# zyhbili/Dual-Space-NeRF

Measured on AMD Instinct MI355X. Metric: rendered rays/sec (64 samples/ray), 512x512 frame, higher is better.
Workload: dtype split-f16x3 (3 x v_mfma_f32_32x32x16_f16 on hi/lo fp16 operand halves, f32 accumulate: f32-equivalent accuracy - parity bars of the tests: 1e-4 absolute on RGB / acc / weights against the reference; sigma 1e-4 absolute where |sigma| <= 100 and 4e-6 RELATIVE to max|sigma| above (this checkpoint: |sig

## Files before the change

dual-space-nerf_amd/csrc/dsn_field16.hip:

```cpp
#include "dsn_common.h"
#include "dsn_kernels.h"

typedef float f32x16 __attribute__((ext_vector_type(16)));
typedef _Float16 half8 __attribute__((ext_vector_type(8)));
#define MFMA16(a, b, c) __builtin_amdgcn_mfma_f32_32x32x16_f16((a), (b), (c), 0, 0, 0)

#if !defined(DSN_EXPERIMENTS) && (defined(F16_ABL) || defined(F16_SABL) || defined(F16_TIMING) || defined(F16_TRAIN_ABL))
#error "F16_ABL / F16_SABL / F16_TIMING are experiment switches (wrong results / debug counters): build with -DDSN_EXPERIMENTS"
#endif
#ifndef F16_SINCOS_OCML
#define F16_SINCOS_OCML 0
#endif
#ifndef F16_FENCE
#define F16_FENCE 0
#endif
#ifndef F16_SGB
#define F16_SGB 1
#endif
#ifndef F16_SGB_VALU
#define F16_SGB_VALU 2
#endif
#ifndef F16_SGB_DS
#define F16_SGB_DS 1
#endif
// ... 1682 lines not shown
        int off = s_base;
        for (int k = 0; k < wave; ++k) off += s_cnt[k];
        if (keep[0]) keep_list[off + __popcll(bm0 & ((1ull << lane) - 1ull))] = (int32_t)pt[0];
        if (keep[1]) keep_list[off + __popcll(bm0) + __popcll(bm1 & ((1ull << lane) - 1ull))] = (int32_t)pt[1];
    }
  }
}

void dsn_launch_screen16(const float* packed, const DsnFrameState* fs, const float* x_c, int64_t N, const int32_t* active_list,
                         const int32_t* active_count, float* sigma, int32_t* keep_list, int32_t* keep_count, float* dbg_sigma,
                         float* dbg_s1, hipStream_t st, int32_t* audit_list, int32_t* audit_count, int audit_cap) {
    if (N == 0) return;
    const char* wenv = getenv("DSN_SCREEN_WAVES");
    const int waves = wenv ? atoi(wenv) : 8;
    static const float margin = getenv("DSN_SCREEN_MARGIN") ? (float)atof(getenv("DSN_SCREEN_MARGIN")) : 0.0f;
    if (waves == 4)
        hipLaunchKernelGGL(k_screen16<4>, dim3((unsigned)std::min<int64_t>((N + 127) / 128, 2 * dsn_cu_count())), dim3(256), 0, st, packed, fs, x_c, N, active_list,
                           active_count, sigma, keep_list, keep_count, dbg_sigma, dbg_s1, margin, audit_list, audit_count, audit_cap);
    else if (waves == 2)
        hipLaunchKernelGGL(k_screen16x2, dim3((unsigned)std::min<int64_t>((N + 255) / 256, dsn_cu_count())), dim3(256), 0, st, packed, fs, x_c, N, active_list,
                           active_count, sigma, keep_list, keep_count, dbg_sigma, dbg_s1, margin, audit_list, audit_count, audit_cap);
    else
        hipLaunchKernelGGL(k_screen16<8>, dim3((unsigned)std::min<int64_t>((N + 255) / 256, dsn_cu_count())), dim3(512), 0, st, packed, fs, x_c, N, active_list,
                           active_count, sigma, keep_list, keep_count, dbg_sigma, dbg_s1, margin, audit_list, audit_count, audit_cap);
}

__global__ void __launch_bounds__(256) k_screen_audit(const int32_t* __restrict__ audit_list, const int32_t* __restrict__ audit_count,
                                                      int audit_cap, const float* __restrict__ sigma, int32_t* __restrict__ out) {
    const int n = min(*audit_count, audit_cap);
    if (blockIdx.x == 0 && threadIdx.x == 0) out[2] = n;
    for (int i = blockIdx.x * 256 + threadIdx.x; i < n; i += gridDim.x * 256) {
        const float s = sigma[audit_list[i]];
        if (s > 0.0f) { atomicAdd(out, 1); atomicMax(out + 1, __float_as_int(s)); }
    }
}
void dsn_launch_screen_audit(const int32_t* audit_list, const int32_t* audit_count, int audit_cap, const float* sigma, int32_t* out,
                             hipStream_t st) {
    hipLaunchKernelGGL(k_screen_audit, dim3(64), dim3(256), 0, st, audit_list, audit_count, audit_cap, sigma, out);
}

#define F16_SCREEN_FLOOR 0.002f
#define F16_SCREEN_CAP 0.15f
#define F16_SCREEN_HEADROOM 10.0f
__global__ void __launch_bounds__(256) k_calib_points(const float4* __restrict__ cent, int F, int64_t n, float* __restrict__ x, float box) {
    const int64_t i = (int64_t)blockIdx.x * 256 + threadIdx.x;
    if (i >= n) return;
    const float4 c = cent[(int)(i % F)];
    uint32_t h = (uint32_t)i * 2654435761u + 0x9e3779b9u;
    float o[3];
    for (int k = 0; k < 3; ++k) {
        h ^= h >> 16; h *= 0x7feb352du; h ^= h >> 15; h *= 0x846ca68bu; h ^= h >> 16;
        o[k] = ((float)(h >> 8) * (1.0f / 16777216.0f) - 0.5f) * box;
    }
    x[3 * i] = c.x + o[0]; x[3 * i + 1] = c.y + o[1]; x[3 * i + 2] = c.z + o[2];
}
#define DSN_CALIB_MIN_FRAME_LIST 65536
__global__ void __launch_bounds__(256) k_calib_points_frame(const float* __restrict__ x_c, const int32_t* __restrict__ list,
                                                             const int32_t* __restrict__ count, const float4* __restrict__ cent, int F,
                                                             int64_t n, float halo, float box, float* __restrict__ x) {
    const int64_t i = (int64_t)blockIdx.x * 256 + threadIdx.x;
    if (i >= n) return;
    const int64_t cnt = (int64_t)(*count);
    uint32_t h = (uint32_t)i * 2654435761u + 0x9e3779b9u;
    float o[3];
    for (int k = 0; k < 3; ++k) {
        h ^= h >> 16; h *= 0x7feb352du; h ^= h >> 15; h *= 0x846ca68bu; h ^= h >> 16;
        o[k] = (float)(h >> 8) * (1.0f / 16777216.0f) - 0.5f;
    }
    if (cnt < DSN_CALIB_MIN_FRAME_LIST) {
        const float4 c = cent[(int)(i % F)];
        x[3 * i] = c.x + o[0] * box; x[3 * i + 1] = c.y + o[1] * box; x[3 * i + 2] = c.z + o[2] * box;
        return;
    }
    const int64_t half = n / 2 > 0 ? n / 2 : 1;
    const int64_t k = i % half;
    const int64_t slot = (int64_t)(((__int128)k * cnt) / half) % cnt;
    const int64_t s = (int64_t)list[slot];
    const float j = i >= half ? 2.0f * halo : 0.0f;
    x[3 * i] = x_c[3 * s] + o[0] * j; x[3 * i + 1] = x_c[3 * s + 1] + o[1] * j; x[3 * i + 2] = x_c[3 * s + 2] + o[2] * j;
}
__global__ void __launch_bounds__(256) k_calib_reduce(const float* __restrict__ sg, const float* __restrict__ s1,
                                                      const float* __restrict__ sig, int64_t n, uint32_t* __restrict__ acc) {
    float d = 0.0f, t = 0.0f;
    int bad = 0;
    for (int64_t i = (int64_t)blockIdx.x * 256 + threadIdx.x; i < n; i += (int64_t)gridDim.x * 256) {
        const float a = sg[i], b = s1[i], c = sig[i];
        const float q = fabsf(a - c) / (b + 1.0f);
        if (q == q && fabsf(q) < INFINITY) {
            d = fmaxf(d, q);
            t = fmaxf(t, q - fabsf(c) / (F16_SCREEN_HEADROOM * (b + 1.0f)));
        } else ++bad;
    }
#pragma unroll
    for (int o = 32; o >= 1; o >>= 1) { d = fmaxf(d, __shfl_xor(d, o)); t = fmaxf(t, __shfl_xor(t, o)); bad += __shfl_xor(bad, o); }
    if ((threadIdx.x & 63) == 0) { atomicMax(acc, __float_as_uint(d)); atomicAdd(acc + 1, (uint32_t)bad); atomicMax(acc + 3, __float_as_uint(t)); }
}
__global__ void k_calib_finish(const uint32_t* __restrict__ acc, float* __restrict__ packed_margin, float* __restrict__ out4, float n) {
    const float d = __uint_as_float(acc[0]);
    float t = __uint_as_float(acc[3]);
    if (out4 && out4[7] > t) t = out4[7];
    float m = fmaxf(F16_SCREEN_HEADROOM * t, F16_SCREEN_FLOOR);
    if (!(m <= F16_SCREEN_CAP)) m = INFINITY;
    *packed_margin = m;
    if (out4) { out4[0] = d; out4[1] = m; out4[2] = (float)acc[1] / n; out4[3] = n; out4[5] = t; }
}
__global__ void __launch_bounds__(256) k_calib_dropped(const float* __restrict__ sg, const float* __restrict__ s1, int64_t n,
                                                       const float* __restrict__ packed_margin, uint32_t* __restrict__ acc) {
    const float m = *packed_margin;
    int c = 0;
    for (int64_t i = (int64_t)blockIdx.x * 256 + threadIdx.x; i < n; i += (int64_t)gridDim.x * 256) c += sg[i] < -(m * s1[i] + m) ? 1 : 0;
#pragma unroll
    for (int o = 32; o >= 1; o >>= 1) c += __shfl_xor(c, o);
    if ((threadIdx.x & 63) == 0 && c) atomicAdd(acc + 2, (uint32_t)c);
}
__global__ void k_calib_dropped_finish(const uint32_t* __restrict__ acc, float* __restrict__ out, float n) { out[4] = (float)acc[2] / n; }
size_t dsn_calibrate_workspace_size(int64_t n) { return 256 + dsn_align256(12 * (size_t)n) + 4 * dsn_align256(4 * (size_t)n); }
void dsn_launch_calibrate_screen(const DsnSceneView& s, float* packed, int64_t n, void* workspace, float* out4, hipStream_t st,
                                 const float* frame_x_c, const int32_t* frame_list, const int32_t* frame_count) {
    char* p = (char*)workspace;
    uint32_t* acc = (uint32_t*)p;             p += 256;
    float* x = (float*)p;                     p += dsn_align256(12 * (size_t)n);
    float* sg = (float*)p;                    p += dsn_align256(4 * (size_t)n);
    float* s1 = (float*)p;                    p += dsn_align256(4 * (size_t)n);
    float* sig = (float*)p;                   p += dsn_align256(4 * (size_t)n);
    int32_t* lst = (int32_t*)p;
    (void)hipMemsetAsync(acc, 0, 256, st);
    const char* be = getenv("DSN_CALIB_BOX");
    const float box = be ? (float)atof(be) : 0.3f;
    if (frame_x_c)
        hipLaunchKernelGGL(k_calib_points_frame, dim3((unsigned)((n + 255) / 256)), dim3(256), 0, st, frame_x_c, frame_list, frame_count,
                           s.cent_canon, s.F, n, 0.02f, box, x);
    else
        hipLaunchKernelGGL(k_calib_points, dim3((unsigned)((n + 255) / 256)), dim3(256), 0, st, s.cent_canon, s.F, n, x, box);
    dsn_launch_screen16(packed, s.frame, x, n, nullptr, nullptr, sg, lst, (int32_t*)(acc + 8), sg, s1, st, nullptr, nullptr, 0);
    dsn_launch_field(packed, s.frame, x, n, nullptr, nullptr, sig, nullptr, nullptr, st);
    hipLaunchKernelGGL(k_calib_reduce, dim3(1024), dim3(256), 0, st, sg, s1, sig, n, acc);
    hipLaunchKernelGGL(k_calib_finish, dim3(1), dim3(1), 0, st, acc, packed + OFF_SCAL + 5, out4, (float)n);
    if (out4) {
        hipLaunchKernelGGL(k_calib_dropped, dim3(1024), dim3(256), 0, st, sg, s1, n, packed + OFF_SCAL + 5, acc);
        hipLaunchKernelGGL(k_calib_dropped_finish, dim3(1), dim3(1), 0, st, acc, out4, (float)n);
    }
}
__global__ void k_set_scalar(float* p, float v) { *p = v; }
void dsn_launch_set_screen_margin(float* packed, float margin, hipStream_t st) {
    hipLaunchKernelGGL(k_set_scalar, dim3(1), dim3(1), 0, st, packed + OFF_SCAL + 5, margin);
}
void dsn_launch_set_packed_scalar(float* packed, int word, float v, hipStream_t st) {
    hipLaunchKernelGGL(k_set_scalar, dim3(1), dim3(1), 0, st, packed + OFF_SCAL + word, v);
}

#define DSN_MFMA(a, b, c) __builtin_amdgcn_mfma_f32_32x32x2f32((a), (b), (c), 0, 0, 0)
__device__ __forceinline__ float dsn_light_mlp32(const float* __restrict__ packed, int lane, const float (&in9)[10]) {
    const int half = lane >> 5;
    f32x16 h1[4], h2[4];
#pragma unroll
    for (int m = 0; m < 4; ++m) {
        f32x16 acc = rows16(packed + OFF_BLT0, m, half);
        const float4* wp = reinterpret_cast<const float4*>(packed + OFF_LT0 + m * DSN_BLK) + lane;
        const float4 w0 = wp[0], w1 = wp[64];
        acc = DSN_MFMA(w0.x, half ? in9[1] : in9[0], acc);
        acc = DSN_MFMA(w0.y, half ? in9[3] : in9[2], acc);
        acc = DSN_MFMA(w0.z, half ? in9[5] : in9[4], acc);
        acc = DSN_MFMA(w0.w, half ? in9[7] : in9[6], acc);
        acc = DSN_MFMA(w1.x, half ? in9[9] : in9[8], acc);
#pragma unroll
        for (int r = 0; r < 16; ++r) acc[r] = acc[r] > 0.0f ? acc[r] : 0.0f;
        h1[m] = acc;
    }
#pragma unroll
    for (int m = 0; m < 4; ++m) {
        f32x16 acc = rows16(packed + OFF_BLT1, m, half);
#pragma unroll
        for (int kb = 0; kb < 4; ++kb) {
            const float4* bp = reinterpret_cast<const float4*>(packed + OFF_LT1 + (m * 4 + kb) * DSN_BLK) + lane;
            const float4 c0 = bp[0], c1 = bp[64], c2 = bp[128], c3 = bp[192];
            acc = DSN_MFMA(c0.x, h1[kb][0], acc);  acc = DSN_MFMA(c0.y, h1[kb][1], acc);
            acc = DSN_MFMA(c0.z, h1[kb][2], acc);  acc = DSN_MFMA(c0.w, h1[kb][3], acc);
            acc = DSN_MFMA(c1.x, h1[kb][4], acc);  acc = DSN_MFMA(c1.y, h1[kb][5], acc);
            acc = DSN_MFMA(c1.z, h1[kb][6], acc);  acc = DSN_MFMA(c1.w, h1[kb][7], acc);
            acc = DSN_MFMA(c2.x, h1[kb][8], acc);  acc = DSN_MFMA(c2.y, h1[kb][9], acc);
            acc = DSN_MFMA(c2.z, h1[kb][10], acc); acc = DSN_MFMA(c2.w, h1[kb][11], acc);
            acc = DSN_MFMA(c3.x, h1[kb][12], acc); acc = DSN_MFMA(c3.y, h1[kb][13], acc);
            acc = DSN_MFMA(c3.z, h1[kb][14], acc); acc = DSN_MFMA(c3.w, h1[kb][15], acc);
        }
#pragma unroll
        for (int r = 0; r < 16; ++r) acc[r] = acc[r] > 0.0f ? acc[r] : 0.0f;
        h2[m] = acc;
    }
    float part = 0.0f;
#pragma unroll
    for (int m = 0; m < 4; ++m) {
        const f32x16 w = rows16(packed + OFF_WLT2, m, half);
#pragma unroll
        for (int r = 0; r < 16; ++r) part = fmaf(w[r], h2[m][r], part);
    }
    part += __shfl_xor(part, 32);
    return part + packed[OFF_SCAL + 4];
}

#define LIGHT32_THREADS 256
__global__ void __launch_bounds__(LIGHT32_THREADS, 1)
k_light(const float* __restrict__ packed, const DsnFrameState* __restrict__ fs, const float* __restrict__ n_w,
        const float* __restrict__ x_w_pts, const float* __restrict__ ray_o, const float* __restrict__ ray_d,
        const float* __restrict__ z_vals, const float* essence, int64_t N, int S,
        const int32_t* __restrict__ active_list, const int32_t* __restrict__ active_count,
        float* colour) {
    DSN_OWN_SIMD();
    const int lane = threadIdx.x & 63;
    const int wave = __builtin_amdgcn_readfirstlane(threadIdx.x >> 6);
    const int half = lane >> 5;
    const int64_t count = active_list ? (int64_t)(*active_count) : N;
    const int64_t slot0 = ((int64_t)blockIdx.x * 4 + wave) * 32;
    if (slot0 >= count) return;
    int64_t slot = slot0 + (lane & 31);
    const bool valid = slot < count;
    if (!valid) slot = count - 1;
    const int64_t pt = active_list ? (int64_t)active_list[slot] : slot;
    const int64_t ray = pt / S;

    float in9[10];
    in9[0] = n_w[3 * pt]; in9[1] = n_w[3 * pt + 1]; in9[2] = n_w[3 * pt + 2];
    float xw[3];
    const float d[3] = {ray_d[3 * ray], ray_d[3 * ray + 1], ray_d[3 * ray + 2]};
    if (x_w_pts) { xw[0] = x_w_pts[3 * pt]; xw[1] = x_w_pts[3 * pt + 1]; xw[2] = x_w_pts[3 * pt + 2]; }
    else {
        const float z = z_vals[pt];
        xw[0] = ray_o[3 * ray] + d[0] * z; xw[1] = ray_o[3 * ray + 1] + d[1] * z; xw[2] = ray_o[3 * ray + 2] + d[2] * z;
    }
    dsn_light_edit(fs->light, xw);
    in9[3] = xw[0]; in9[4] = xw[1]; in9[5] = xw[2];
    const float vn = dsn_norm3(d);
    in9[6] = dsn_div(d[0], vn); in9[7] = dsn_div(d[1], vn); in9[8] = dsn_div(d[2], vn);
    in9[9] = 0.0f;

    const float o = dsn_light_mlp32(packed, lane, in9);
    const float wgt = (o > 0.0f ? o : expm1f(o)) + 1.0f;
    if (valid && half == 0) {
        colour[3 * pt + 0] = wgt * essence[3 * pt + 0];
        colour[3 * pt + 1] = wgt * essence[3 * pt + 1];
        colour[3 * pt + 2] = wgt * essence[3 * pt + 2];
    }
}

void dsn_launch_light(const float* packed, const DsnFrameState* fs, const float* n_w, const float* x_w,
                      const float* ray_o, const float* ray_d, const float* z_vals, const float* essence, int64_t N,
                      int S, const int32_t* active_list, const int32_t* active_count, float* colour, hipStream_t st) {
    int64_t blocks = (N + 127) / 128;
    if (blocks == 0) return;
    hipLaunchKernelGGL(k_light, dim3((unsigned)blocks), dim3(LIGHT32_THREADS), 0, st, packed, fs, n_w, x_w, ray_o, ray_d,
                       z_vals, essence, N, S, active_list, active_count, colour);
}

__device__ __forceinline__ void light_block0(const char* blkp, int lane, const half8 (&xh)[2], const half8 (&xl)[2], f32x16& aM, f32x16& aC) {
    const half8 h0 = *reinterpret_cast<const half8*>(blkp + lane * 16);
    const half8 l0 = *reinterpret_cast<const half8*>(blkp + 1024 + lane * 16);
    aM = MFMA16(h0, xh[0], aM);
    aC = MFMA16(h0, xl[0], aC);
    aC = MFMA16(l0, xh[0], aC);
}
__device__ __forceinline__ void light_block(const char* __restrict__ blkp, int lane, const half8 (&xh)[2], const half8 (&xl)[2],
                                            f32x16& aM, f32x16& aC, bool second_step) {
    const half8 h0 = *reinterpret_cast<const half8*>(blkp + lane * 16);
    const half8 l0 = *reinterpret_cast<const half8*>(blkp + 1024 + lane * 16);
    aM = MFMA16(h0, xh[0], aM);
    aC = MFMA16(h0, xl[0], aC);
    aC = MFMA16(l0, xh[0], aC);
    if (second_step) {
        const half8 h1 = *reinterpret_cast<const half8*>(blkp + 2048 + lane * 16);
        const half8 l1 = *reinterpret_cast<const half8*>(blkp + 3072 + lane * 16);
        aM = MFMA16(h1, xh[1], aM);
        aC = MFMA16(h1, xl[1], aC);
        aC = MFMA16(l1, xh[1], aC);
    }
}

#define LIGHT_LDS_BYTES (4 * 2048 + 16 * 4096)
__device__ __forceinline__ void light16_stage_weights(const float* __restrict__ packed, char* s_w) {
    const char* g16 = reinterpret_cast<const char*>(packed + OFF16_BASE);
    const uint4* g0 = reinterpret_cast<const uint4*>(g16 + (size_t)(OFF_LT0 / DSN_BLK) * 4096);
    const uint4* g1 = reinterpret_cast<const uint4*>(g16 + (size_t)(OFF_LT1 / DSN_BLK) * 4096);
    uint4* d = reinterpret_cast<uint4*>(s_w);
    for (int i = threadIdx.x; i < 4 * 128; i += 256) d[i] = g0[(i >> 7) * 256 + (i & 127)];
    for (int i = threadIdx.x; i < 16 * 256; i += 256) d[4 * 128 + i] = g1[i];
    __syncthreads();
}
struct LightIn { float nw[3], o[3], d[3], z; };
__device__ __forceinline__ int64_t light16_tile_slot(int64_t t, int wave, int lane, int64_t ntiles, int64_t count, bool& ok) {
    int64_t sl = (t * 4 + wave) * 32 + (lane & 31);
    ok = t < ntiles && sl < count;
    if (!ok) sl = count - 1;
    return sl;
}
__device__ __forceinline__ void light16_fetch(int64_t p, int S, const float* __restrict__ n_w, const float* __restrict__ x_w_pts,
                                              const float* __restrict__ ray_o, const float* __restrict__ ray_d,
                                              const float* __restrict__ z_vals, LightIn& a) {
    const int64_t r = p / S;
    a.nw[0] = n_w[3 * p]; a.nw[1] = n_w[3 * p + 1]; a.nw[2] = n_w[3 * p + 2];
    a.d[0] = ray_d[3 * r]; a.d[1] = ray_d[3 * r + 1]; a.d[2] = ray_d[3 * r + 2];
    if (x_w_pts) { a.o[0] = x_w_pts[3 * p]; a.o[1] = x_w_pts[3 * p + 1]; a.o[2] = x_w_pts[3 * p + 2]; a.z = 0.0f; }
    else { a.o[0] = ray_o[3 * r]; a.o[1] = ray_o[3 * r + 1]; a.o[2] = ray_o[3 * r + 2]; a.z = z_vals[p]; }
}
__device__ __forceinline__ float light16_mlp(const float* __restrict__ packed, const char* s_w, int lane, const float (&in9)[10],
                                             bool valid, int64_t pt, float* __restrict__ tr_hl1, float* __restrict__ tr_hl2,
                                             bool& flagged) {
    const int half = lane >> 5;
    float ovf = packed[DSN_SPLIT_UNSAFE_LIGHT];
    half8 xh[2], xl[2];
    {
        f32x16 v = zero16();
#pragma unroll
        for (int j = 0; j < 5; ++j) v[j] = half ? in9[2 * j + 1] : in9[2 * j];
        track16(ovf, v);
        split16<true>(v, xh, xl);
    }
    half8 h1h[4][2], h1l[4][2];
#pragma unroll
    for (int m = 0; m < 4; ++m) {
        f32x16 aM = rows16(packed + OFF_BLT0, m, half), aC = zero16();
        light_block0(s_w + m * 2048, lane, xh, xl, aM, aC);
        f32x16 v = fold16(aM, aC);
#pragma unroll
        for (int r = 0; r < 16; ++r) v[r] = fmaxf(v[r], 0.0f);
        if (tr_hl1 && valid) store16(tr_hl1 + pt * 128 + 4 * half + 32 * m, v, 1.0f);
        track16(ovf, v);
        split16<true>(v, h1h[m], h1l[m]);
    }
    float part = 0.0f;
#pragma unroll
    for (int m = 0; m < 4; ++m) {
        f32x16 aM = rows16(packed + OFF_BLT1, m, half), aC = zero16();
#pragma unroll
        for (int kb = 0; kb < 4; ++kb)
            light_block(s_w + 4 * 2048 + (m * 4 + kb) * 4096, lane, h1h[kb], h1l[kb], aM, aC, true);
        f32x16 v = fold16(aM, aC);
        const f32x16 w2 = rows16(packed + OFF_WLT2, m, half);
#pragma unroll
        for (int r = 0; r < 16; ++r) { v[r] = fmaxf(v[r], 0.0f); part = fmaf(w2[r], v[r], part); }
        if (tr_hl2 && valid) store16(tr_hl2 + pt * 128 + 4 * half + 32 * m, v, 1.0f);
    }
    part += __shfl_xor(part, 32);
    float o = part + packed[OFF_SCAL + 4];
    flagged = !(fmaxf(ovf, __shfl_xor(ovf, 32)) < F16_RANGE_SCALED);
    if (__ballot(flagged)) {
        const float e = dsn_light_mlp32(packed, lane, in9);
        if (flagged) o = e;
    }
    return o;
}
__device__ __forceinline__ float light16_weight(float o) { return (o > 0.0f ? o : expm1f(o)) + 1.0f; }

template <bool FACTOR>
__global__ void __launch_bounds__(256, 1)
k_light16(const float* __restrict__ packed, const DsnFrameState* __restrict__ fs, const float* __restrict__ n_w,
          const float* __restrict__ x_w_pts, const float* __restrict__ ray_o, const float* __restrict__ ray_d,
          const float* __restrict__ z_vals, const float* essence, int64_t N, int S,
          const int32_t* __restrict__ active_list, const int32_t* __restrict__ active_count,
          float* colour, float* __restrict__ tr_hl1, float* __restrict__ tr_hl2, float* __restrict__ tr_pre,
          int32_t* __restrict__ range_count, float* __restrict__ factor) {
    __shared__ __attribute__((aligned(16))) char s_w[LIGHT_LDS_BYTES];
#ifndef F16_SHARE_SIMD
    DSN_OWN_SIMD();
#endif
    const int lane = threadIdx.x & 63;
    const int wave = __builtin_amdgcn_readfirstlane(threadIdx.x >> 6);
    const int half = lane >> 5;
    const int64_t count = active_list ? (int64_t)(*active_count) : N;
    const int64_t ntiles = (count + 127) / 128;
    if ((int64_t)blockIdx.x >= ntiles) return;
    light16_stage_weights(packed, s_w);
    auto tile_pt = [&](int64_t t, bool& ok) -> int64_t {
        const int64_t sl = light16_tile_slot(t, wave, lane, ntiles, count, ok);
        return active_list ? (int64_t)active_list[sl] : sl;
    };
    bool valid_c, valid_n, valid_nn;
    int64_t pt_c = tile_pt(blockIdx.x, valid_c);
    LightIn in_c, in_n;
    light16_fetch(pt_c, S, n_w, x_w_pts, ray_o, ray_d, z_vals, in_c);
    int64_t pt_n = tile_pt((int64_t)blockIdx.x + gridDim.x, valid_n);
  for (int64_t tile = blockIdx.x; tile < ntiles; tile += gridDim.x) {
    const int64_t slot0 = (tile * 4 + wave) * 32;
    const bool valid = valid_c;
    const int64_t pt = pt_c;
    const LightIn cur = in_c;
    light16_fetch(pt_n, S, n_w, x_w_pts, ray_o, ray_d, z_vals, in_n);
    const int64_t pt_nn = tile_pt(tile + 2 * (int64_t)gridDim.x, valid_nn);
    pt_c = pt_n; valid_c = valid_n; in_c = in_n;
    pt_n = pt_nn; valid_n = valid_nn;
    if (slot0 >= count) continue;
    const float ess[3] = {essence[3 * pt], essence[3 * pt + 1], essence[3 * pt + 2]};

    float in9[10];
    in9[0] = cur.nw[0]; in9[1] = cur.nw[1]; in9[2] = cur.nw[2];
    float xw[3];
    const float d[3] = {cur.d[0], cur.d[1], cur.d[2]};
    if (x_w_pts) { xw[0] = cur.o[0]; xw[1] = cur.o[1]; xw[2] = cur.o[2]; }
    else {
        const float z = cur.z;
        xw[0] = cur.o[0] + d[0] * z; xw[1] = cur.o[1] + d[1] * z; xw[2] = cur.o[2] + d[2] * z;
    }
    dsn_light_edit(fs->light, xw);
    in9[3] = xw[0]; in9[4] = xw[1]; in9[5] = xw[2];
    const float vn = dsn_norm3(d);
    in9[6] = dsn_div(d[0], vn); in9[7] = dsn_div(d[1], vn); in9[8] = dsn_div(d[2], vn);
    in9[9] = 0.0f;

    bool flagged;
    const float o = light16_mlp(packed, s_w, lane, in9, valid, pt, tr_hl1, tr_hl2, flagged);
    if (flagged && range_count && valid && half == 0) atomicAdd(range_count, 1);
    const float wgt = light16_weight(o);
    if (tr_pre && valid && half == 0) tr_pre[pt] = o;
    if (valid && half == 0) {
        colour[3 * pt + 0] = wgt * ess[0];
        colour[3 * pt + 1] = wgt * ess[1];
        colour[3 * pt + 2] = wgt * ess[2];
        if (FACTOR) factor[pt] = wgt;
    }
  }
}

void dsn_launch_light16(const float* packed, const DsnFrameState* fs, const float* n_w, const float* x_w,
                        const float* ray_o, const float* ray_d, const float* z_vals, const float* essence, int64_t N,
                        int S, const int32_t* active_list, const int32_t* active_count, float* colour, hipStream_t st,
                        float* tr_hl1, float* tr_hl2, float* tr_pre, int32_t* range_count, float* factor) {
    int64_t blocks = (N + 127) / 128;
    if (blocks == 0) return;
    const dim3 grid((unsigned)std::min<int64_t>(blocks, (int64_t)dsn_cu_count()));
    if (factor)
        hipLaunchKernelGGL(k_light16<true>, grid, dim3(256), 0, st, packed, fs, n_w, x_w, ray_o, ray_d, z_vals, essence, N, S, active_list,
                           active_count, colour, tr_hl1, tr_hl2, tr_pre, range_count, factor);
    else
        hipLaunchKernelGGL(k_light16<false>, grid, dim3(256), 0, st, packed, fs, n_w, x_w, ray_o, ray_d, z_vals, essence, N, S, active_list,
                           active_count, colour, tr_hl1, tr_hl2, tr_pre, range_count, factor);
}

template <bool FACTOR>
__global__ void __launch_bounds__(256, 1)
k_light16_multi(const float* __restrict__ packed, const DsnLightEdit* __restrict__ lights, int G, const float* __restrict__ n_w,
                const float* __restrict__ ray_o, const float* __restrict__ ray_d, const float* __restrict__ z_vals,
                const float* __restrict__ essence, int S, const int32_t* __restrict__ list, const int32_t* __restrict__ list_count,
                float* __restrict__ colours, float* __restrict__ factors) {
    __shared__ __attribute__((aligned(16))) char s_w[LIGHT_LDS_BYTES];
#ifndef F16_SHARE_SIMD
    DSN_OWN_SIMD();
#endif
    const int lane = threadIdx.x & 63;
    const int wave = __builtin_amdgcn_readfirstlane(threadIdx.x >> 6);
    const int half = lane >> 5;
    const int64_t count = *list_count;
    const int64_t ntiles = (count + 127) / 128;
    if ((int64_t)blockIdx.x >= ntiles) return;
    light16_stage_weights(packed, s_w);
    auto tile_pt = [&](int64_t t, bool& ok) -> int64_t { return (int64_t)list[light16_tile_slot(t, wave, lane, ntiles, count, ok)]; };
    bool valid_c, valid_n, valid_nn;
    int64_t pt_c = tile_pt(blockIdx.x, valid_c);
    LightIn in_c, in_n;
    light16_fetch(pt_c, S, n_w, nullptr, ray_o, ray_d, z_vals, in_c);
    int64_t pt_n = tile_pt((int64_t)blockIdx.x + gridDim.x, valid_n);
  for (int64_t tile = blockIdx.x; tile < ntiles; tile += gridDim.x) {
    const int64_t slot0 = (tile * 4 + wave) * 32;
    const int64_t slot = slot0 + (lane & 31);
    const bool valid = valid_c;
    const int64_t pt = pt_c;
    const LightIn cur = in_c;
    light16_fetch(pt_n, S, n_w, nullptr, ray_o, ray_d, z_vals, in_n);
    const int64_t pt_nn = tile_pt(tile + 2 * (int64_t)gridDim.x, valid_nn);
    pt_c = pt_n; valid_c = valid_n; in_c = in_n;
    pt_n = pt_nn; valid_n = valid_nn;
    if (slot0 >= count) continue;
    const float ess[3] = {essence[3 * pt], essence[3 * pt + 1], essence[3 * pt + 2]};
    const float d[3] = {cur.d[0], cur.d[1], cur.d[2]};
    float xw0[3];
    {
        const float z = cur.z;
        xw0[0] = cur.o[0] + d[0] * z; xw0[1] = cur.o[1] + d[1] * z; xw0[2] = cur.o[2] + d[2] * z;
    }
    const float vn = dsn_norm3(d);
    const float vd[3] = {dsn_div(d[0], vn), dsn_div(d[1], vn), dsn_div(d[2], vn)};
    for (int g = 0; g < G; ++g) {
        asm volatile("" ::: "memory");
        float in9[10];
        in9[0] = cur.nw[0]; in9[1] = cur.nw[1]; in9[2] = cur.nw[2];
        float xw[3] = {xw0[0], xw0[1], xw0[2]};
        dsn_light_edit(lights[g], xw);
        in9[3] = xw[0]; in9[4] = xw[1]; in9[5] = xw[2];
        in9[6] = vd[0]; in9[7] = vd[1]; in9[8] = vd[2];
        in9[9] = 0.0f;
        bool flagged;
        const float wgt = light16_weight(light16_mlp(packed, s_w, lane, in9, valid, pt, nullptr, nullptr, flagged));
        if (valid && half == 0) {
            float* c = colours + ((int64_t)g * count + slot) * 3;
            c[0] = wgt * ess[0];
            c[1] = wgt * ess[1];
            c[2] = wgt * ess[2];
            if (FACTOR) factors[(int64_t)g * count + slot] = wgt;
        }
    }
  }
}

void dsn_launch_light16_multi(const float* packed, const DsnLightEdit* lights, int G, const float* n_w, const float* ray_o, const float* ray_d,
                              const float* z_vals, const float* essence, int64_t max_count, int S, const int32_t* list,
                              const int32_t* list_count, float* colours, hipStream_t st, float* factors) {
    const int64_t blocks = (max_count + 127) / 128;
    if (blocks == 0 || G < 1) return;
    const dim3 grid((unsigned)std::min<int64_t>(blocks, (int64_t)dsn_cu_count()));
    if (factors)
        hipLaunchKernelGGL(k_light16_multi<true>, grid, dim3(256), 0, st, packed, lights, G, n_w, ray_o, ray_d, z_vals, essence, S, list,
                           list_count, colours, factors);
    else
        hipLaunchKernelGGL(k_light16_multi<false>, grid, dim3(256), 0, st, packed, lights, G, n_w, ray_o, ray_d, z_vals, essence, S, list,
                           list_count, colours, factors);
}
```

Baseline: 31.50 million.

## Process two light-MLP tiles per wave with software-pipelined MFMA and epilogue scheduling

Restructures the fp16-split light MLP so each wave evaluates two tiles (or two lights in the multi-light kernel) at once. It shares each LDS weight read across both tiles and prefetches the next weight block. sched_group_barriers interleave MFMAs with the previous layer's epilogue VALU work, and biases and scalars are staged into LDS. The goal is to hide MFMA latency and cut redundant weight and global scalar loads, at the cost of higher register pressure, a more complex schedule, and a fallback path that now refetches inputs.

```diff
diff --git a/dual-space-nerf_amd/csrc/dsn_field16.hip b/dual-space-nerf_amd/csrc/dsn_field16.hip
--- a/dual-space-nerf_amd/csrc/dsn_field16.hip
+++ b/dual-space-nerf_amd/csrc/dsn_field16.hip
@@ -1858,7 +1858,7 @@
 #define DSN_MFMA(a, b, c) __builtin_amdgcn_mfma_f32_32x32x2f32((a), (b), (c), 0, 0, 0)
 __device__ __forceinline__ float dsn_light_mlp32(const float* __restrict__ packed, int lane, const float (&in9)[10]) {
     const int half = lane >> 5;
-    f32x16 h1[4], h2[4];
+    f32x16 h1[4];
 #pragma unroll
     for (int m = 0; m < 4; ++m) {
         f32x16 acc = rows16(packed + OFF_BLT0, m, half);
@@ -1873,6 +1873,7 @@
         for (int r = 0; r < 16; ++r) acc[r] = acc[r] > 0.0f ? acc[r] : 0.0f;
         h1[m] = acc;
     }
+    float part = 0.0f;
 #pragma unroll
     for (int m = 0; m < 4; ++m) {
         f32x16 acc = rows16(packed + OFF_BLT1, m, half);
@@ -1891,14 +1892,9 @@
         }
 #pragma unroll
         for (int r = 0; r < 16; ++r) acc[r] = acc[r] > 0.0f ? acc[r] : 0.0f;
-        h2[m] = acc;
-    }
-    float part = 0.0f;
-#pragma unroll
-    for (int m = 0; m < 4; ++m) {
         const f32x16 w = rows16(packed + OFF_WLT2, m, half);
 #pragma unroll
-        for (int r = 0; r < 16; ++r) part = fmaf(w[r], h2[m][r], part);
+        for (int r = 0; r < 16; ++r) part = fmaf(w[r], acc[r], part);
     }
     part += __shfl_xor(part, 32);
     return part + packed[OFF_SCAL + 4];
@@ -1957,30 +1953,57 @@
                        z_vals, essence, N, S, active_list, active_count, colour);
 }
 
-__device__ __forceinline__ void light_block0(const char* blkp, int lane, const half8 (&xh)[2], const half8 (&xl)[2], f32x16& aM, f32x16& aC) {
-    const half8 h0 = *reinterpret_cast<const half8*>(blkp + lane * 16);
-    const half8 l0 = *reinterpret_cast<const half8*>(blkp + 1024 + lane * 16);
-    aM = MFMA16(h0, xh[0], aM);
-    aC = MFMA16(h0, xl[0], aC);
-    aC = MFMA16(l0, xh[0], aC);
-}
-__device__ __forceinline__ void light_block(const char* __restrict__ blkp, int lane, const half8 (&xh)[2], const half8 (&xl)[2],
-                                            f32x16& aM, f32x16& aC, bool second_step) {
-    const half8 h0 = *reinterpret_cast<const half8*>(blkp + lane * 16);
-    const half8 l0 = *reinterpret_cast<const half8*>(blkp + 1024 + lane * 16);
-    aM = MFMA16(h0, xh[0], aM);
-    aC = MFMA16(h0, xl[0], aC);
-    aC = MFMA16(l0, xh[0], aC);
-    if (second_step) {
-        const half8 h1 = *reinterpret_cast<const half8*>(blkp + 2048 + lane * 16);
-        const half8 l1 = *reinterpret_cast<const half8*>(blkp + 3072 + lane * 16);
-        aM = MFMA16(h1, xh[1], aM);
-        aC = MFMA16(h1, xl[1], aC);
-        aC = MFMA16(l1, xh[1], aC);
-    }
-}
-
-#define LIGHT_LDS_BYTES (4 * 2048 + 16 * 4096)
+struct LightW { half8 h0, l0, h1, l1; };
+__device__ __forceinline__ LightW light_wread(const char* s_w, int lane, int id) {
+    LightW w;
+    const char* p = s_w + (id < 4 ? id * 2048 : 4 * 2048 + (id - 4) * 4096) + lane * 16;
+    w.h0 = *reinterpret_cast<const half8*>(p);
+    w.l0 = *reinterpret_cast<const half8*>(p + 1024);
+    if (id < 4) { w.h1 = w.h0; w.l1 = w.l0; }
+    else { w.h1 = *reinterpret_cast<const half8*>(p + 2048); w.l1 = *reinterpret_cast<const half8*>(p + 3072); }
+    return w;
+}
+template <int NT>
+__device__ __forceinline__ void light_block0(const LightW& w, const half8 (&xh)[NT][2], const half8 (&xl)[NT][2], f32x16 (&aM)[NT], f32x16 (&aC)[NT]) {
+#pragma unroll
+    for (int t = 0; t < NT; ++t) aM[t] = MFMA16(w.h0, xh[t][0], aM[t]);
+#pragma unroll
+    for (int t = 0; t < NT; ++t) aC[t] = MFMA16(w.h0, xl[t][0], aC[t]);
+#pragma unroll
+    for (int t = 0; t < NT; ++t) aC[t] = MFMA16(w.l0, xh[t][0], aC[t]);
+}
+__device__ __forceinline__ void light_block_tile(const LightW& w, const half8 (&xh)[2], const half8 (&xl)[2], f32x16& aM, f32x16& aC) {
+    aM = MFMA16(w.h0, xh[0], aM);
+    aC = MFMA16(w.h0, xl[0], aC);
+    aC = MFMA16(w.l0, xh[0], aC);
+    aM = MFMA16(w.h1, xh[1], aM);
+    aC = MFMA16(w.h1, xl[1], aC);
+    aC = MFMA16(w.l1, xh[1], aC);
+}
+template <int NT, bool BY_TILE>
+__device__ __forceinline__ void light_block(const LightW& w, const half8 (&xh)[NT][2], const half8 (&xl)[NT][2], f32x16 (&aM)[NT], f32x16 (&aC)[NT]) {
+    if (BY_TILE) {
+#pragma unroll
+        for (int t = 0; t < NT; ++t) light_block_tile(w, xh[t], xl[t], aM[t], aC[t]);
+        return;
+    }
+    light_block0<NT>(w, xh, xl, aM, aC);
+#pragma unroll
+    for (int t = 0; t < NT; ++t) aM[t] = MFMA16(w.h1, xh[t][1], aM[t]);
+#pragma unroll
+    for (int t = 0; t < NT; ++t) aC[t] = MFMA16(w.h1, xl[t][1], aC[t]);
+#pragma unroll
+    for (int t = 0; t < NT; ++t) aC[t] = MFMA16(w.l1, xh[t][1], aC[t]);
+}
+
+#define LIGHT_W_BYTES (4 * 2048 + 16 * 4096)
+#define LIGHT_C_BLT0 0
+#define LIGHT_C_BLT1 128
+#define LIGHT_C_WLT2 256
+#define LIGHT_C_BOUT 384
+#define LIGHT_C_UNSAFE 385
+#define LIGHT_C_FLOATS 392
+#define LIGHT_LDS_BYTES (LIGHT_W_BYTES + 4 * LIGHT_C_FLOATS)
 __device__ __forceinline__ void light16_stage_weights(const float* __restrict__ packed, char* s_w) {
     const char* g16 = reinterpret_cast<const char*>(packed + OFF16_BASE);
     const uint4* g0 = reinterpret_cast<const uint4*>(g16 + (size_t)(OFF_LT0 / DSN_BLK) * 4096);
@@ -1988,6 +2011,10 @@
     uint4* d = reinterpret_cast<uint4*>(s_w);
     for (int i = threadIdx.x; i < 4 * 128; i += 256) d[i] = g0[(i >> 7) * 256 + (i & 127)];
     for (int i = threadIdx.x; i < 16 * 256; i += 256) d[4 * 128 + i] = g1[i];
+    float* c = reinterpret_cast<float*>(s_w + LIGHT_W_BYTES);
+    for (int i = threadIdx.x; i < LIGHT_C_FLOATS; i += 256)
+        c[i] = i < 128 ? packed[OFF_BLT0 + i] : i < 256 ? packed[OFF_BLT1 + (i - 128)] : i < 384 ? packed[OFF_WLT2 + (i - 256)]
+             : i == LIGHT_C_BOUT ? packed[OFF_SCAL + 4] : i == LIGHT_C_UNSAFE ? packed[DSN_SPLIT_UNSAFE_LIGHT] : 0.0f;
     __syncthreads();
 }
 struct LightIn { float nw[3], o[3], d[3], z; };
@@ -2006,56 +2033,203 @@
     if (x_w_pts) { a.o[0] = x_w_pts[3 * p]; a.o[1] = x_w_pts[3 * p + 1]; a.o[2] = x_w_pts[3 * p + 2]; a.z = 0.0f; }
     else { a.o[0] = ray_o[3 * r]; a.o[1] = ray_o[3 * r + 1]; a.o[2] = ray_o[3 * r + 2]; a.z = z_vals[p]; }
 }
-__device__ __forceinline__ float light16_mlp(const float* __restrict__ packed, const char* s_w, int lane, const float (&in9)[10],
-                                             bool valid, int64_t pt, float* __restrict__ tr_hl1, float* __restrict__ tr_hl2,
-                                             bool& flagged) {
+#define LIGHT_SGB_VALU1 8
+#define LIGHT_SGB_VALU13 6
+template <int NT, bool TR>
+__device__ __forceinline__ float light16_mlp(const char* s_w, int lane, const float (&in9)[NT][10], const bool (&valid)[NT],
+                                            const int64_t (&pt)[NT], float* __restrict__ tr_hl1, float* __restrict__ tr_hl2,
+                                            bool (&flagged)[NT], float (&o)[NT]) {
     const int half = lane >> 5;
-    float ovf = packed[DSN_SPLIT_UNSAFE_LIGHT];
-    half8 xh[2], xl[2];
-    {
+    const float* s_c = reinterpret_cast<const float*>(s_w + LIGHT_W_BYTES);
+    asm volatile("" ::: "memory");
+    float ovf[NT];
+    half8 xh[NT][2], xl[NT][2];
+#pragma unroll
+    for (int t = 0; t < NT; ++t) {
+        ovf[t] = s_c[LIGHT_C_UNSAFE];
         f32x16 v = zero16();
 #pragma unroll
-        for (int j = 0; j < 5; ++j) v[j] = half ? in9[2 * j + 1] : in9[2 * j];
-        track16(ovf, v);
-        split16<true>(v, xh, xl);
-    }
-    half8 h1h[4][2], h1l[4][2];
+        for (int j = 0; j < 5; ++j) v[j] = half ? in9[t][2 * j + 1] : in9[t][2 * j];
+        track16(ovf[t], v);
+        split16<true>(v, xh[t], xl[t]);
+    }
+    int si = 0;
+    LightW wn = light_wread(s_w, lane, 0);
+    auto take = [&]() __attribute__((always_inline)) {
+        const LightW w = wn;
+        ++si;
+        if (si < 20) wn = light_wread(s_w, lane, si);
+        return w;
+    };
+    half8 h1h[4][NT][2], h1l[4][NT][2];
+    f32x16 a1M[2][NT], a1C[2][NT], a2M[NT], a2C[NT];
+    auto mfma1 = [&](int m) __attribute__((always_inline)) {
+        const f32x16 b = rows16(s_c + LIGHT_C_BLT0, m, half);
+#pragma unroll
+        for (int t = 0; t < NT; ++t) { a1M[m & 1][t] = b; a1C[m & 1][t] = zero16(); }
+        light_block0<NT>(take(), xh, xl, a1M[m & 1], a1C[m & 1]);
+    };
+    auto mfma2 = [&](int m, int kb) __attribute__((always_inline)) {
+        if (kb == 0) {
+            const f32x16 b = rows16(s_c + LIGHT_C_BLT1, m, half);
+#pragma unroll
+            for (int t = 0; t < NT; ++t) { a2M[t] = b; a2C[t] = zero16(); }
+        }
+        if (kb == 0 || kb == 3) light_block<NT, true>(take(), h1h[kb], h1l[kb], a2M, a2C);
+        else light_block<NT, false>(take(), h1h[kb], h1l[kb], a2M, a2C);
+    };
+    auto epi1 = [&](int m) __attribute__((always_inline)) {
+#pragma unroll
+        for (int t = 0; t < NT; ++t) {
+            f32x16 v = fold16(a1M[m & 1][t], a1C[m & 1][t]);
+#pragma unroll
+            for (int r = 0; r < 16; ++r) v[r] = fmaxf(v[r], 0.0f);
+            if (TR) { if (tr_hl1 && valid[t]) store16(tr_hl1 + pt[t] * 128 + 4 * half + 32 * m, v, 1.0f); }
+            track16(ovf[t], v);
+            split16<true>(v, h1h[m][t], h1l[m][t]);
+        }
+    };
+    float part[NT];
+#pragma unroll
+    for (int t = 0; t < NT; ++t) part[t] = 0.0f;
+    auto epi2 = [&](int m, int t) __attribute__((always_inline)) {
+        f32x16 v = fold16(a2M[t], a2C[t]);
+        const f32x16 w2 = rows16(s_c + LIGHT_C_WLT2, m, half);
+#pragma unroll
+        for (int r = 0; r < 16; ++r) { v[r] = fmaxf(v[r], 0.0f); part[t] = fmaf(w2[r], v[r], part[t]); }
+        if (TR) { if (tr_hl2 && valid[t]) store16(tr_hl2 + pt[t] * 128 + 4 * half + 32 * m, v, 1.0f); }
+    };
+    mfma1(0);
+    __builtin_amdgcn_sched_barrier(0);
+#pragma unroll
+    for (int k = 0; k < 3; ++k) {
+        mfma1(k + 1);
+        epi1(k);
+#pragma unroll
+        for (int i = 0; i < 3 * NT; ++i) {
+            __builtin_amdgcn_sched_group_barrier(0x008, 1, 0);
+            __builtin_amdgcn_sched_group_barrier(0x002, LIGHT_SGB_VALU1, 0);
+        }
+        __builtin_amdgcn_sched_barrier(0);
+    }
+    mfma2(0, 0); mfma2(0, 1); mfma2(0, 2);
+    epi1(3);
+#pragma unroll
+    for (int i = 0; i < 18 * NT; ++i) {
+        __builtin_amdgcn_sched_group_barrier(0x008, 1, 0);
+        __builtin_amdgcn_sched_group_barrier(0x002, LIGHT_SGB_VALU13, 0);
+    }
+    __builtin_amdgcn_sched_barrier(0);
 #pragma unroll
     for (int m = 0; m < 4; ++m) {
-        f32x16 aM = rows16(packed + OFF_BLT0, m, half), aC = zero16();
-        light_block0(s_w + m * 2048, lane, xh, xl, aM, aC);
-        f32x16 v = fold16(aM, aC);
-#pragma unroll
-        for (int r = 0; r < 16; ++r) v[r] = fmaxf(v[r], 0.0f);
-        if (tr_hl1 && valid) store16(tr_hl1 + pt * 128 + 4 * half + 32 * m, v, 1.0f);
-        track16(ovf, v);
-        split16<true>(v, h1h[m], h1l[m]);
-    }
-    float part = 0.0f;
-#pragma unroll
-    for (int m = 0; m < 4; ++m) {
-        f32x16 aM = rows16(packed + OFF_BLT1, m, half), aC = zero16();
-#pragma unroll
-        for (int kb = 0; kb < 4; ++kb)
-            light_block(s_w + 4 * 2048 + (m * 4 + kb) * 4096, lane, h1h[kb], h1l[kb], aM, aC, true);
-        f32x16 v = fold16(aM, aC);
-        const f32x16 w2 = rows16(packed + OFF_WLT2, m, half);
-#pragma unroll
-        for (int r = 0; r < 16; ++r) { v[r] = fmaxf(v[r], 0.0f); part = fmaf(w2[r], v[r], part); }
-        if (tr_hl2 && valid) store16(tr_hl2 + pt * 128 + 4 * half + 32 * m, v, 1.0f);
-    }
-    part += __shfl_xor(part, 32);
-    float o = part + packed[OFF_SCAL + 4];
-    flagged = !(fmaxf(ovf, __shfl_xor(ovf, 32)) < F16_RANGE_SCALED);
-    if (__ballot(flagged)) {
-        const float e = dsn_light_mlp32(packed, lane, in9);
-        if (flagged) o = e;
-    }
-    return o;
+        if (m > 0) {
+            if (NT == 2) epi2(m - 1, NT - 1);
+            mfma2(m, 0);
+            if (NT == 2) {
+#pragma unroll
+                for (int i = 0; i < 6; ++i) {
+                    __builtin_amdgcn_sched_group_barrier(0x008, 1, 0);
+                    __builtin_amdgcn_sched_group_barrier(0x002, LIGHT_SGB_VALU1, 0);
+                }
+            }
+            __builtin_amdgcn_sched_barrier(0);
+            mfma2(m, 1);
+            __builtin_amdgcn_sched_barrier(0);
+            mfma2(m, 2);
+            __builtin_amdgcn_sched_barrier(0);
+        }
+        mfma2(m, 3);
+        epi2(m, 0);
+        if (NT == 2) {
+#pragma unroll
+            for (int i = 0; i < 6; ++i) __builtin_amdgcn_sched_group_barrier(0x008, 1, 0);
+#pragma unroll
+            for (int i = 0; i < 6; ++i) {
+                __builtin_amdgcn_sched_group_barrier(0x008, 1, 0);
+                __builtin_amdgcn_sched_group_barrier(0x002, LIGHT_SGB_VALU1, 0);
+            }
+        }
+        __builtin_amdgcn_sched_barrier(0);
+    }
+    if (NT == 2) epi2(3, NT - 1);
+#pragma unroll
+    for (int t = 0; t < NT; ++t) {
+        part[t] += __shfl_xor(part[t], 32);
+        o[t] = part[t] + s_c[LIGHT_C_BOUT];
+        flagged[t] = !(fmaxf(ovf[t], __shfl_xor(ovf[t], 32)) < F16_RANGE_SCALED);
+    }
+    return o[0];
+}
+__device__ __forceinline__ void light16_fallback(const float* __restrict__ packed, int lane, const float (&in9)[10], bool flagged, float& o) {
+    const float* p = packed;
+    asm volatile("" : "+s"(p));
+    const float e = dsn_light_mlp32(p, lane, in9);
+    if (flagged) o = e;
 }
 __device__ __forceinline__ float light16_weight(float o) { return (o > 0.0f ? o : expm1f(o)) + 1.0f; }
 
-template <bool FACTOR>
+__device__ __forceinline__ void light16_in9(const LightIn& a, bool world, const DsnLightEdit& light, float (&in9)[10]) {
+    in9[0] = a.nw[0]; in9[1] = a.nw[1]; in9[2] = a.nw[2];
+    float xw[3];
+    const float d[3] = {a.d[0], a.d[1], a.d[2]};
+    if (world) { xw[0] = a.o[0]; xw[1] = a.o[1]; xw[2] = a.o[2]; }
+    else {
+        const float z = a.z;
+        xw[0] = a.o[0] + d[0] * z; xw[1] = a.o[1] + d[1] * z; xw[2] = a.o[2] + d[2] * z;
+    }
+    dsn_light_edit(light, xw);
+    in9[3] = xw[0]; in9[4] = xw[1]; in9[5] = xw[2];
+    const float vn = dsn_norm3(d);
+    in9[6] = dsn_div(d[0], vn); in9[7] = dsn_div(d[1], vn); in9[8] = dsn_div(d[2], vn);
+    in9[9] = 0.0f;
+}
+__device__ __forceinline__ bool light16_has_second(int64_t tile, int64_t G, int wave, int64_t ntiles, int64_t count) {
+    return tile + G < ntiles && ((tile + G) * 4 + wave) * 32 < count;
+}
+struct LightSrc { const float *n_w, *x_w_pts, *ray_o, *ray_d, *z_vals; int S; };
+template <int NT, bool FACTOR, bool TRAIN>
+__device__ __forceinline__ void light16_trip(const float* __restrict__ packed, const char* s_w, int lane, const DsnLightEdit& light, const LightSrc& src,
+                                             const LightIn (&cur)[2], const int64_t (&pt2)[2], const bool (&valid2)[2],
+                                             const float* essence, float* colour, float* __restrict__ tr_hl1, float* __restrict__ tr_hl2,
+                                             float* __restrict__ tr_pre, int32_t* __restrict__ range_count, float* __restrict__ factor) {
+    const int half = lane >> 5;
+    float ess[NT][3], in9[NT][10], o[NT];
+    bool valid[NT], flagged[NT];
+    int64_t pt[NT];
+#pragma unroll
+    for (int t = 0; t < NT; ++t) {
+        valid[t] = valid2[t]; pt[t] = pt2[t];
+        ess[t][0] = essence[3 * pt[t]]; ess[t][1] = essence[3 * pt[t] + 1]; ess[t][2] = essence[3 * pt[t] + 2];
+        light16_in9(cur[t], src.x_w_pts != nullptr, light, in9[t]);
+    }
+    light16_mlp<NT, TRAIN>(s_w, lane, in9, valid, pt, tr_hl1, tr_hl2, flagged, o);
+#pragma unroll 1
+    for (int t = 0; t < NT; ++t) {
+        const bool second = NT == 2 && t == 1;
+        const bool f = second ? flagged[NT - 1] : flagged[0];
+        if (__ballot(f)) {
+            LightIn a;
+            light16_fetch(second ? pt[NT - 1] : pt[0], src.S, src.n_w, src.x_w_pts, src.ray_o, src.ray_d, src.z_vals, a);
+            float x9[10];
+            light16_in9(a, src.x_w_pts != nullptr, light, x9);
+            if (second) light16_fallback(packed, lane, x9, f, o[NT - 1]); else light16_fallback(packed, lane, x9, f, o[0]);
+        }
+    }
+#pragma unroll
+    for (int t = 0; t < NT; ++t) {
+        if (flagged[t] && range_count && valid[t] && half == 0) atomicAdd(range_count, 1);
+        const float wgt = light16_weight(o[t]);
+        if (tr_pre && valid[t] && half == 0) tr_pre[pt[t]] = o[t];
+        if (valid[t] && half == 0) {
+            colour[3 * pt[t] + 0] = wgt * ess[t][0];
+            colour[3 * pt[t] + 1] = wgt * ess[t][1];
+            colour[3 * pt[t] + 2] = wgt * ess[t][2];
+            if (FACTOR) factor[pt[t]] = wgt;
+        }
+    }
+}
+
+template <bool FACTOR, bool TRAIN>
 __global__ void __launch_bounds__(256, 1)
 k_light16(const float* __restrict__ packed, const DsnFrameState* __restrict__ fs, const float* __restrict__ n_w,
           const float* __restrict__ x_w_pts, const float* __restrict__ ray_o, const float* __restrict__ ray_d,
@@ -2069,58 +2243,52 @@
 #endif
     const int lane = threadIdx.x & 63;
     const int wave = __builtin_amdgcn_readfirstlane(threadIdx.x >> 6);
-    const int half = lane >> 5;
     const int64_t count = active_list ? (int64_t)(*active_count) : N;
     const int64_t ntiles = (count + 127) / 128;
     if ((int64_t)blockIdx.x >= ntiles) return;
     light16_stage_weights(packed, s_w);
+    const int64_t G = gridDim.x;
+    const LightSrc src = {n_w, x_w_pts, ray_o, ray_d, z_vals, S};
     auto tile_pt = [&](int64_t t, bool& ok) -> int64_t {
+        if (t >= ntiles) { ok = false; return 0; }
         const int64_t sl = light16_tile_slot(t, wave, lane, ntiles, count, ok);
         return active_list ? (int64_t)active_list[sl] : sl;
     };
-    bool valid_c, valid_n, valid_nn;
-    int64_t pt_c = tile_pt(blockIdx.x, valid_c);
-    LightIn in_c, in_n;
-    light16_fetch(pt_c, S, n_w, x_w_pts, ray_o, ray_d, z_vals, in_c);
-    int64_t pt_n = tile_pt((int64_t)blockIdx.x + gridDim.x, valid_n);
-  for (int64_t tile = blockIdx.x; tile < ntiles; tile += gridDim.x) {
-    const int64_t slot0 = (tile * 4 + wave) * 32;
-    const bool valid = valid_c;
-    const int64_t pt = pt_c;
-    const LightIn cur = in_c;
-    light16_fetch(pt_n, S, n_w, x_w_pts, ray_o, ray_d, z_vals, in_n);
-    const int64_t pt_nn = tile_pt(tile + 2 * (int64_t)gridDim.x, valid_nn);
-    pt_c = pt_n; valid_c = valid_n; in_c = in_n;
-    pt_n = pt_nn; valid_n = valid_nn;
-    if (slot0 >= count) continue;
-    const float ess[3] = {essence[3 * pt], essence[3 * pt + 1], essence[3 * pt + 2]};
-
-    float in9[10];
-    in9[0] = cur.nw[0]; in9[1] = cur.nw[1]; in9[2] = cur.nw[2];
-    float xw[3];
-    const float d[3] = {cur.d[0], cur.d[1], cur.d[2]};
-    if (x_w_pts) { xw[0] = cur.o[0]; xw[1] = cur.o[1]; xw[2] = cur.o[2]; }
-    else {
-        const float z = cur.z;
-        xw[0] = cur.o[0] + d[0] * z; xw[1] = cur.o[1] + d[1] * z; xw[2] = cur.o[2] + d[2] * z;
-    }
-    dsn_light_edit(fs->light, xw);
-    in9[3] = xw[0]; in9[4] = xw[1]; in9[5] = xw[2];
-    const float vn = dsn_norm3(d);
-    in9[6] = dsn_div(d[0], vn); in9[7] = dsn_div(d[1], vn); in9[8] = dsn_div(d[2], vn);
-    in9[9] = 0.0f;
-
-    bool flagged;
-    const float o = light16_mlp(packed, s_w, lane, in9, valid, pt, tr_hl1, tr_hl2, flagged);
-    if (flagged && range_count && valid && half == 0) atomicAdd(range_count, 1);
-    const float wgt = light16_weight(o);
-    if (tr_pre && valid && half == 0) tr_pre[pt] = o;
-    if (valid && half == 0) {
-        colour[3 * pt + 0] = wgt * ess[0];
-        colour[3 * pt + 1] = wgt * ess[1];
-        colour[3 * pt + 2] = wgt * ess[2];
-        if (FACTOR) factor[pt] = wgt;
-    }
+    auto fetch = [&](int64_t t, int64_t p, LightIn& a) { if (t < ntiles) light16_fetch(p, S, n_w, x_w_pts, ray_o, ray_d, z_vals, a); };
+    bool valid_c[2], valid_n[2], valid_nn[2];
+    int64_t pt_c[2], pt_n[2], pt_nn[2];
+    LightIn in_c[2] = {}, in_n[2] = {};
+#pragma unroll
+    for (int i = 0; i < 2; ++i) {
+        pt_c[i] = tile_pt(blockIdx.x + i * G, valid_c[i]);
+        fetch(blockIdx.x + i * G, pt_c[i], in_c[i]);
+    }
+#pragma unroll
+    for (int i = 0; i < 2; ++i) pt_n[i] = tile_pt(blockIdx.x + (2 + i) * G, valid_n[i]);
+  for (int64_t tile = blockIdx.x; tile < ntiles; tile += 2 * G) {
+    const bool valid[2] = {valid_c[0], valid_c[1]};
+    const int64_t pt[2] = {pt_c[0], pt_c[1]};
+    const LightIn cur[2] = {in_c[0], in_c[1]};
+#pragma unroll
+    for (int i = 0; i < 2; ++i) {
+        fetch(tile + (2 + i) * G, pt_n[i], in_n[i]);
+        pt_nn[i] = tile_pt(tile + (4 + i) * G, valid_nn[i]);
+        pt_c[i] = pt_n[i]; valid_c[i] = valid_n[i]; in_c[i] = in_n[i];
+        pt_n[i] = pt_nn[i]; valid_n[i] = valid_nn[i];
+    }
+    if ((tile * 4 + wave) * 32 >= count) continue;
+    if constexpr (TRAIN) {
+        light16_trip<1, FACTOR, TRAIN>(packed, s_w, lane, fs->light, src, cur, pt, valid, essence, colour, tr_hl1, tr_hl2, tr_pre, range_count, factor);
+        if (light16_has_second(tile, G, wave, ntiles, count)) {
+            const LightIn cur1[2] = {cur[1], cur[1]};
+            const int64_t pt1[2] = {pt[1], pt[1]};
+            const bool valid1[2] = {valid[1], valid[1]};
+            light16_trip<1, FACTOR, TRAIN>(packed, s_w, lane, fs->light, src, cur1, pt1, valid1, essence, colour, tr_hl1, tr_hl2, tr_pre, range_count, factor);
+        }
+    } else if (light16_has_second(tile, G, wave, ntiles, count))
+        light16_trip<2, FACTOR, TRAIN>(packed, s_w, lane, fs->light, src, cur, pt, valid, essence, colour, tr_hl1, tr_hl2, tr_pre, range_count, factor);
+    else
+        light16_trip<1, FACTOR, TRAIN>(packed, s_w, lane, fs->light, src, cur, pt, valid, essence, colour, tr_hl1, tr_hl2, tr_pre, range_count, factor);
   }
 }
 
@@ -2131,12 +2299,55 @@
     int64_t blocks = (N + 127) / 128;
     if (blocks == 0) return;
     const dim3 grid((unsigned)std::min<int64_t>(blocks, (int64_t)dsn_cu_count()));
-    if (factor)
-        hipLaunchKernelGGL(k_light16<true>, grid, dim3(256), 0, st, packed, fs, n_w, x_w, ray_o, ray_d, z_vals, essence, N, S, active_list,
-                           active_count, colour, tr_hl1, tr_hl2, tr_pre, range_count, factor);
-    else
-        hipLaunchKernelGGL(k_light16<false>, grid, dim3(256), 0, st, packed, fs, n_w, x_w, ray_o, ray_d, z_vals, essence, N, S, active_list,
-                           active_count, colour, tr_hl1, tr_hl2, tr_pre, range_count, factor);
+    auto k = tr_hl1 || tr_hl2 ? (factor ? k_light16<true, true> : k_light16<false, true>) : (factor ? k_light16<true, false> : k_light16<false, false>);
+    hipLaunchKernelGGL(k, grid, dim3(256), 0, st, packed, fs, n_w, x_w, ray_o, ray_d, z_vals, essence, N, S, active_list,
+                       active_count, colour, tr_hl1, tr_hl2, tr_pre, range_count, factor);
+}
+
+struct LightFix { float nw[3], xw0[3], vd[3]; };
+__device__ __forceinline__ void light16_multi_in9(const LightFix& q, const DsnLightEdit& light, float (&in9)[10]) {
+    in9[0] = q.nw[0]; in9[1] = q.nw[1]; in9[2] = q.nw[2];
+    float xw[3] = {q.xw0[0], q.xw0[1], q.xw0[2]};
+    dsn_light_edit(light, xw);
+    in9[3] = xw[0]; in9[4] = xw[1]; in9[5] = xw[2];
+    in9[6] = q.vd[0]; in9[7] = q.vd[1]; in9[8] = q.vd[2];
+    in9[9] = 0.0f;
+}
+template <int NT, bool FACTOR>
+__device__ __forceinline__ void light16_multi_step(const float* __restrict__ packed, const char* s_w, int lane, const DsnLightEdit* __restrict__ lights,
+                                                   int g, const LightFix& fx, const float (&ess)[3], bool valid1, int64_t pt1, int64_t slot,
+                                                   int64_t count, float* __restrict__ colours, float* __restrict__ factors) {
+    const int half = lane >> 5;
+    float in9[NT][10], o[NT];
+    bool valid[NT], flagged[NT];
+    int64_t pt[NT];
+#pragma unroll
+    for (int t = 0; t < NT; ++t) {
+        valid[t] = valid1; pt[t] = pt1;
+        light16_multi_in9(fx, lights[g + t], in9[t]);
+    }
+    light16_mlp<NT, false>(s_w, lane, in9, valid, pt, nullptr, nullptr, flagged, o);
+#pragma unroll 1
+    for (int t = 0; t < NT; ++t) {
+        const bool second = NT == 2 && t == 1;
+        const bool f = second ? flagged[NT - 1] : flagged[0];
+        if (__ballot(f)) {
+            float x9[10];
+            light16_multi_in9(fx, lights[g + t], x9);
+            if (second) light16_fallback(packed, lane, x9, f, o[NT - 1]); else light16_fallback(packed, lane, x9, f, o[0]);
+        }
+    }
+#pragma unroll
+    for (int t = 0; t < NT; ++t) {
+        const float wgt = light16_weight(o[t]);
+        if (valid1 && half == 0) {
+            float* c = colours + ((int64_t)(g + t) * count + slot) * 3;
+            c[0] = wgt * ess[0];
+            c[1] = wgt * ess[1];
+            c[2] = wgt * ess[2];
+            if (FACTOR) factors[(int64_t)(g + t) * count + slot] = wgt;
+        }
+    }
 }
 
 template <bool FACTOR>
@@ -2151,7 +2362,6 @@
 #endif
     const int lane = threadIdx.x & 63;
     const int wave = __builtin_amdgcn_readfirstlane(threadIdx.x >> 6);
-    const int half = lane >> 5;
     const int64_t count = *list_count;
     const int64_t ntiles = (count + 127) / 128;
     if ((int64_t)blockIdx.x >= ntiles) return;
@@ -2174,32 +2384,18 @@
     pt_n = pt_nn; valid_n = valid_nn;
     if (slot0 >= count) continue;
     const float ess[3] = {essence[3 * pt], essence[3 * pt + 1], essence[3 * pt + 2]};
-    const float d[3] = {cur.d[0], cur.d[1], cur.d[2]};
-    float xw0[3];
+    LightFix fx;
     {
+        const float d[3] = {cur.d[0], cur.d[1], cur.d[2]};
         const float z = cur.z;
-        xw0[0] = cur.o[0] + d[0] * z; xw0[1] = cur.o[1] + d[1] * z; xw0[2] = cur.o[2] + d[2] * z;
-    }
-    const float vn = dsn_norm3(d);
-    const float vd[3] = {dsn_div(d[0], vn), dsn_div(d[1], vn), dsn_div(d[2], vn)};
-    for (int g = 0; g < G; ++g) {
-        asm volatile("" ::: "memory");
-        float in9[10];
-        in9[0] = cur.nw[0]; in9[1] = cur.nw[1]; in9[2] = cur.nw[2];
-        float xw[3] = {xw0[0], xw0[1], xw0[2]};
-        dsn_light_edit(lights[g], xw);
-        in9[3] = xw[0]; in9[4] = xw[1]; in9[5] = xw[2];
-        in9[6] = vd[0]; in9[7] = vd[1]; in9[8] = vd[2];
-        in9[9] = 0.0f;
-        bool flagged;
-        const float wgt = light16_weight(light16_mlp(packed, s_w, lane, in9, valid, pt, nullptr, nullptr, flagged));
-        if (valid && half == 0) {
-            float* c = colours + ((int64_t)g * count + slot) * 3;
-            c[0] = wgt * ess[0];
-            c[1] = wgt * ess[1];
-            c[2] = wgt * ess[2];
-            if (FACTOR) factors[(int64_t)g * count + slot] = wgt;
-        }
+        fx.xw0[0] = cur.o[0] + d[0] * z; fx.xw0[1] = cur.o[1] + d[1] * z; fx.xw0[2] = cur.o[2] + d[2] * z;
+        const float vn = dsn_norm3(d);
+        fx.vd[0] = dsn_div(d[0], vn); fx.vd[1] = dsn_div(d[1], vn); fx.vd[2] = dsn_div(d[2], vn);
+        fx.nw[0] = cur.nw[0]; fx.nw[1] = cur.nw[1]; fx.nw[2] = cur.nw[2];
+    }
+    for (int g = 0; g < G; g += 2) {
+        if (g + 1 < G) light16_multi_step<2, FACTOR>(packed, s_w, lane, lights, g, fx, ess, valid, pt, slot, count, colours, factors);
+        else light16_multi_step<1, FACTOR>(packed, s_w, lane, lights, g, fx, ess, valid, pt, slot, count, colours, factors);
     }
   }
 }
```

Result: no change. 31.80 million (median of 4 runs) (+0.9%).
